# david-jk/BigGAN-Tensorflow

Measured on AMD Instinct MI355X. Metric: BigGAN-128 train-step images/sec, higher is better.
Workload: dtype bf16; 1 GPU; BigGAN-128 ch=96 bf16 (BASELINE config 3: global batch 256, 32/GPU over 8 GPUs); img_size=128, ch=96, per_gpu_batch=256, global_batch=256, da_policy=full, g_regularization=ortho_cosine, n_labels=0, gan_type=hinge, hip_graph=False, precision=bf16, parallelism=dp1

## Files before the change

### biggan-tensorflow_amd/csrc/igemm16.hip

```cpp
#include <stdlib.h>

#include "common.h"
#include "igemm.h"
#include "igemm16.h"
#include <type_traits>
#include "igemm_dev.h"

namespace bg {

typedef float f32x4_t __attribute__((ext_vector_type(4)));
typedef float f32x16_t __attribute__((ext_vector_type(16)));
typedef __bf16 bf16x8_t __attribute__((ext_vector_type(8)));
typedef short s16x4v __attribute__((ext_vector_type(4)));
typedef short s16x8v __attribute__((ext_vector_type(8)));
typedef __attribute__((address_space(3))) void lds_void_t;
typedef __attribute__((address_space(1))) const void gbl_void_t;
typedef __attribute__((address_space(3))) s16x4v lds_s16x4v;

__device__ uint4 g_zero_page[1024];

__device__ __forceinline__ void glds16(const void* src, unsigned char* lds_wave_base) {
    __builtin_amdgcn_global_load_lds((gbl_void_t*)src, (lds_void_t*)lds_wave_base, 16, 0, 0);
}

__device__ __forceinline__ void glds16_asm(const void* src, uint32_t lds_byte_addr) {
    unsigned keep;
    const uint32_t dst = __builtin_amdgcn_readfirstlane(lds_byte_addr);
    asm volatile("s_mov_b32 %0, m0\n\ts_mov_b32 m0, %2\n\ts_nop 0\n\tglobal_load_lds_dwordx4 %1, off\n\ts_mov_b32 m0, %0"
                 : "=&s"(keep)
                 : "v"(src), "s"(dst)
                 : "memory");
}

__device__ __forceinline__ uint32_t pack_bf16x2(float a, float b) {
    typedef __bf16 bf16x2_t __attribute__((ext_vector_type(2)));
    bf16x2_t v;
    v[0] = (__bf16)a;
    v[1] = (__bf16)b;
    return __builtin_bit_cast(uint32_t, v);
}
__device__ __forceinline__ float bf16_lo(uint32_t u) { return __builtin_bit_cast(float, u << 16); }
__device__ __forceinline__ float bf16_hi(uint32_t u) { return __builtin_bit_cast(float, u & 0xffff0000u); }

constexpr int NN16_BM = 128;
constexpr int NN16_TAPS = 4;
constexpr int NN16_RING_TAPS = 8;
constexpr int nn16_lds_bytes(int TN, int TAPS = NN16_TAPS) {
    const int stage = (NN16_BM + 32 * TN) * 128;
    const int epi = NN16_BM * (32 * TN + 4) * 4;
    const int tab = 2 * TAPS * NN16_BM * 4;
    return (2 * stage + tab > epi ? 2 * stage + tab : epi) + NN16_BM * 4 + 16;
}
constexpr int nn16_pipe_lds_bytes(int TN, int WM, int TAPS = NN16_TAPS) {
    const int bm = 64 * WM;
    return 3 * (bm + 32 * TN) * 64 + TAPS * bm * (4 + 2) + bm * 4 + 16;
}
constexpr int NN16_NOSRC = -(1 << 30);

template <int MODE>
__device__ __forceinline__ int64_t nn16_src_off(const Gather& g, const RowPos& r, int kh, int kw) {
    int h, w;
    if (MODE == GATHER_CONV) {
        h = conv_src(r.ho, kh, g.stride, g.pad, g.reflect, g.Hs);
        w = conv_src(r.wo, kw, g.stride, g.pad, g.reflect, g.Ws);
    } else {
        h = tconv_src_from_num(r.ho + g.pad - kh, g.stride, g.Hs);
        w = tconv_src_from_num(r.wo + g.pad - kw, g.stride, g.Ws);
    }
    const bool ok = r.valid && h >= 0 && w >= 0;
    const int pix = (r.b * g.Hs + h) * g.Ws + w;
    return ok ? (int64_t)pix * g.ld : (int64_t)-1;
}

constexpr int NN16_NOMIRROR = -(1 << 20);
__device__ __forceinline__ int nn16_mirror_pos(int o, int n, bool hi) {
    return o == 1 ? -1 : ((hi && o == n - 2) ? n : NN16_NOMIRROR);
}

template <int MODE, bool PM, bool RING = false>
__device__ __forceinline__ RowPos nn16_row(const NN16Params& p, int m, int ph, int pw) {
    RowPos r;
    if (PM) {
        r.valid = m < p.M;
        const int pos = m / p.g.Nb;
        r.b = m - pos * p.g.Nb;
        if (RING) {
            const int L = p.ring_lines, first = L * p.g.Wo;
            if (pos < first) {
                const int line = pos / p.g.Wo;
                r.ho = line == 0 ? 1 : p.g.Ho - 2;
                r.wo = pos - line * p.g.Wo;
            } else {
                const int per = p.g.Ho - L, q = pos - first;
                const int line = q / per, idx = q - line * per;
                r.wo = line == 0 ? 1 : p.g.Wo - 2;
                r.ho = idx == 0 ? 0 : ((L == 2 && idx > p.g.Ho - 4) ? p.g.Ho - 1 : idx + 1);
            }
            return r;
        }
        const int hq = pos / p.g.Wq;
        r.ho = hq * p.g.pstep + ph;
        r.wo = (pos - hq * p.g.Wq) * p.g.pstep + pw;
        return r;
    }
    if (MODE == GATHER_PLAIN || !p.pow2) return decompose_row<MODE>(p.g, m, p.M, ph, pw);
    r.valid = m < p.M;
    const int wq = m & (p.g.Wq - 1);
    const int t = m >> p.wq_shift;
    const int hq = t & (p.g.Hq - 1);
    r.b = t >> p.hq_shift;
    r.ho = hq * p.g.pstep + ph;
    r.wo = wq * p.g.pstep + pw;
    return r;
}

template <int TN, int MODE, bool PM, bool RING = false, int SLOTS = 2, int WM = 2>
__global__ __launch_bounds__(128 * WM, SLOTS == 2 ? 2 : (WM == 4 ? 4 : 3)) void nn16_kernel(const NN16Params p) {
    static_assert(!RING || (PM && MODE == GATHER_TCONV), "ring launches are position-major transposed gathers");
    static_assert((SLOTS == 2 && WM == 2) || (SLOTS == 3 && (WM == 2 || WM == 4)), "two stages, or a 3-slot ring on 4 / 8 waves");
    constexpr bool PIPE = SLOTS == 3;
    constexpr int TAPS = RING ? NN16_RING_TAPS : NN16_TAPS;
    constexpr int LDS_BYTES = PIPE ? nn16_pipe_lds_bytes(TN, WM, TAPS) : nn16_lds_bytes(TN, TAPS);
    typedef typename std::conditional<RING, uint64_t, unsigned>::type mask_t;
    typedef typename std::conditional<PIPE, int16_t, int>::type tabw_t;
    constexpr int BM = 64 * WM, BN = 32 * TN, NTHR = 128 * WM, NWV = 2 * WM;
    constexpr int CPS = PIPE ? 4 : 8;
    constexpr int ROWB = 16 * CPS;
    constexpr int RSTR = PIPE ? 16 * NWV : 32;
    constexpr int JA = BM / RSTR, JB = PIPE ? (BN / 16 + NWV - 1) / NWV : BN / 32;
    constexpr int A_BYTES = BM * ROWB, STAGE = (BM + BN) * ROWB;
    static_assert(BM == NN16_BM || PIPE, "the two-stage form has 128-row tiles");
    static_assert(A_BYTES % 1024 == 0 && STAGE % 1024 == 0 && (RSTR * ROWB) % 1024 == 0,
                  "every LDS-DMA destination is 1 KB aligned");
    static_assert(!PIPE || 64 * (BN + 4) * 4 <= SLOTS * STAGE, "a 64-row part of the epilogue fits in front of the tables");
    static_assert(!PIPE || RING || LDS_BYTES * (WM == 4 ? 2 : 3) <= 160 * 1024, "ring forms: 3 (8 waves: 2) blocks per CU");
    static_assert(!PIPE || LDS_BYTES * 2 <= 160 * 1024, "mirrored-tap ring launches: 2 blocks per CU");
    extern __shared__ __attribute__((aligned(16))) unsigned char smem[];

    const int t = threadIdx.x;
    const int lane = t & 63, w = PIPE ? __builtin_amdgcn_readfirstlane(t >> 6) : t >> 6;
    const int wm = w >> 1, wn = w & 1;
    const Gather& g = p.g;

    int tile_m, tile_n, bz = blockIdx.z;
    if (p.zfold > 0) {
        const int lin = xcd_remap(blockIdx.x, p.tiles_m * p.tiles_n * p.zfold);
        if (p.mfast) {
            tile_m = lin % p.tiles_m;
            const int r_ = lin / p.tiles_m;
            bz = r_ % p.zfold;
            tile_n = r_ / p.zfold;
        } else {
            bz = lin % p.zfold;
            const int tile = lin / p.zfold;
            tile_n = tile % p.tiles_n;
            tile_m = tile / p.tiles_n;
        }
    } else {
        const int tile = xcd_remap(blockIdx.x, p.tiles_m * p.tiles_n);
        if (p.mfast) {
            tile_m = tile % p.tiles_m;
            tile_n = tile / p.tiles_m;
        } else {
            tile_n = tile % p.tiles_n;
            tile_m = tile / p.tiles_n;
        }
    }
    const int m0 = tile_m * BM, n0 = tile_n * BN;
    const int zs = bz % p.splitk, zo = bz / p.splitk;

    int ph = 0, pw = 0;
    if (MODE == GATHER_TCONV) {
        ph = g.pstep - 1 - zo / g.pstep;
        pw = g.pstep - 1 - zo % g.pstep;
    }
    int kh0 = 0, kw0 = 0, kstep = 1, nkh = g.k, nkw = g.k;
    if (MODE == GATHER_TCONV && g.pstep > 1) {
        kstep = g.stride;
        kh0 = (ph + g.pad) % g.stride;
        kw0 = (pw + g.pad) % g.stride;
        nkh = (g.k - kh0 + g.stride - 1) / g.stride;
        nkw = (g.k - kw0 + g.stride - 1) / g.stride;
    }
    int nrh = 0, nrw = 0;
    if (RING) {
        nrh = nrw = g.k;
        nkh = nkw = 2 * g.k;
    }
    const int C8 = p.C >> 3;
    const int ntap = nkh * nkw;

    unsigned& s_any = *reinterpret_cast<unsigned*>(smem + LDS_BYTES - 16);
    if (PM) {
        if (t == 0) s_any = 0;
        __syncthreads();
    }
    unsigned any_local = 0;
    int* tabh = reinterpret_cast<int*>(smem + SLOTS * STAGE);
    tabw_t* tabw = reinterpret_cast<tabw_t*>(tabh + TAPS * BM);
    for (int e = t; e < 2 * TAPS * BM; e += NTHR) {
        const int axis = e / (TAPS * BM), i = (e / BM) % TAPS, row = e % BM;
        const RowPos r = nn16_row<MODE, PM, RING>(p, m0 + row, ph, pw);
        int v = NN16_NOSRC;
        if (r.valid && i < (axis ? nkw : nkh)) {
            int kk = (axis ? kw0 : kh0) + i * kstep;
            int o = axis ? r.wo : r.ho;
            const int n = axis ? g.Ws : g.Hs;
            if (RING) {
                const int nr = axis ? nrw : nrh;
                if (i >= nr) {
                    kk = i - nr;
                    o = nn16_mirror_pos(o, axis ? g.Wo : g.Ho, p.ring_lines == 2);
                }
            }
            const int src = MODE == GATHER_CONV ? conv_src(o, kk, g.stride, g.pad, g.reflect, n)
                                                : (o == NN16_NOMIRROR ? -1 : tconv_src_from_num(o + g.pad - kk, g.stride, n));
            if (src >= 0) {
                v = axis ? src : (r.b * g.Hs + src) * g.Ws;
                any_local |= 1u << (axis * TAPS + i);
            }
        }
        if (PIPE && axis) tabw[e - TAPS * BM] = (tabw_t)(v < 0 ? -1 : v);
        else tabh[e] = v;
    }
    if (PM && any_local) atomicOr(&s_any, any_local);
    unsigned* tabo = reinterpret_cast<unsigned*>(smem + LDS_BYTES - 16 - BM * 4);
    constexpr bool use_tabo = MODE == GATHER_TCONV || PM;
    if (use_tabo && t < BM) {
        const RowPos r = nn16_row<MODE, PM, RING>(p, m0 + t, ph, pw);
        tabo[t] = (r.valid && r.ho < g.Ho && r.wo < g.Wo) ? (unsigned)((r.b * g.Ho + r.ho) * g.Wo + r.wo) : 0xffffffffu;
    }

    const int cch = PIPE ? (lane & 3) ^ ((lane >> 3) & 2) : (lane & 7) ^ ((((w & 1) << 2) | (lane >> 4)) & 7);
    const int rsub = PIPE ? 16 * w + (lane >> 2) : 8 * w + (lane >> 3);
    constexpr int NB_HI = JB, NB_LO = (BN / 16) / NWV;
    const int nbw = (PIPE && NB_HI != NB_LO) ? (BN / 16 - w + NWV - 1) / NWV : JB;
    const unsigned char* abase = reinterpret_cast<const unsigned char*>(p.A);
    const unsigned char* bbase = reinterpret_cast<const unsigned char*>(p.B);
    const unsigned char* zero = reinterpret_cast<const unsigned char*>(g_zero_page);
    const unsigned ald2 = 2u * (unsigned)g.ld;
    const uint32_t lds0 = static_cast<uint32_t>(
        reinterpret_cast<uintptr_t>((__attribute__((address_space(3))) unsigned char*)smem));

    __syncthreads();
    mask_t tapmask = 0;
    if (PM) {
        const unsigned any = __builtin_amdgcn_readfirstlane(s_any);
        for (int i = 0; i < nkh; ++i)
            for (int j = 0; j < nkw; ++j)
                if (((any >> i) & (any >> (TAPS + j)) & 1u) != 0 && !(RING && i < nrh && j < nrw))
                    tapmask |= (mask_t)1 << (i * TAPS + j);
    }
    const int nsteps_all = ((PM ? __builtin_popcountll((uint64_t)tapmask) : ntap) * C8 + 7) >> 3;
    const int sps = (nsteps_all + p.splitk - 1) / p.splitk;
    const int it0 = zs * sps;
    const int nsteps = max(0, min(nsteps_all, it0 + sps) - it0);

    mask_t rem = tapmask;
    int tidx = 0, c8, ih = 0, iw = 0;
    {
        const int kk = it0 * 8 + cch;
        tidx = kk / C8;
        c8 = kk - tidx * C8;
        if (PM) {
            for (int i = 0; i < tidx && rem; ++i) rem &= rem - 1;
        } else {
            ih = tidx / nkw;
            iw = tidx - ih * nkw;
        }
    }
    const unsigned char* asrc[JA];
    const unsigned char* wsrc[JB];
    auto set_tap = [&]() {
        bool kvalid;
        if (PM) {
            kvalid = rem != 0;
            const int bit = kvalid ? __builtin_ctzll((uint64_t)rem) : 0;
            ih = bit / TAPS;
            iw = bit % TAPS;
        } else {
            kvalid = tidx < ntap;
        }
        const int* th = tabh + (ih & (TAPS - 1)) * BM + rsub;
        const tabw_t* tw = tabw + (iw & (TAPS - 1)) * BM + rsub;
#pragma unroll
        for (int j = 0; j < JA; ++j) {
            int col = tw[RSTR * j];
            if (PIPE) col = col < 0 ? NN16_NOSRC : col;
            const int pix = th[RSTR * j] + col;
            asrc[j] = (kvalid & (pix >= 0)) ? abase + (uint64_t)(unsigned)pix * ald2 : zero;
        }
        const int kh = RING ? (ih >= nrh ? ih - nrh : ih) : kh0 + ih * kstep;
        const int kw = RING ? (iw >= nrw ? iw - nrw : iw) : kw0 + iw * kstep;
        const unsigned char* wt = bbase + 2 * (int64_t)(kh * g.k + kw) * p.tap_stride;
#pragma unroll
        for (int j = 0; j < JB; ++j) {
            const int n = n0 + RSTR * j + rsub;
            wsrc[j] = (kvalid & (n < p.N)) ? wt + 2 * (uint64_t)((unsigned)n * (unsigned)p.C) : zero;
        }
    };
    set_tap();
    auto advance = [&]() {
        c8 += CPS;
        if (c8 >= C8) {
            do {
                c8 -= C8;
                if (PM) {
                    rem &= rem - 1;
                } else {
                    ++tidx;
                    if (++iw == nkw) {
                        iw = 0;
                        ++ih;
                    }
                }
            } while (c8 >= C8);
            set_tap();
        }
    };

    auto stage = [&](int buf) {
        const uint32_t sa = lds0 + buf * STAGE + w * 1024;
        const uint32_t sb = sa + A_BYTES;
        const unsigned cbyte = 16u * (unsigned)c8;
#pragma unroll
        for (int j = 0; j < JA; ++j) glds16_asm(asrc[j] + cbyte, sa + j * RSTR * ROWB);
#pragma unroll
        for (int j = 0; j < JB; ++j)
            if (!PIPE || j < nbw) glds16_asm(wsrc[j] + cbyte, sb + j * RSTR * ROWB);
        advance();
    };

    f32x4_t acc[4][TN];
#pragma unroll
    for (int i = 0; i < 4; ++i)
#pragma unroll
        for (int j = 0; j < TN; ++j)
#pragma unroll
            for (int r = 0; r < 4; ++r) acc[i][j][r] = 0.f;

    if constexpr (PIPE) {
        const int frag = (lane & 15) * ROWB + 16 * ((lane >> 4) ^ (((lane & 15) >> 1) & 2));
        const unsigned char* a_ad = smem + wm * 64 * ROWB + frag;
        const unsigned char* b_ad = smem + A_BYTES + wn * 16 * TN * ROWB + frag;
        const int nst = 2 * nsteps;
        if (nst > 0) stage(0);
        if (nst > 1) stage(1);
        auto kstep = [&](int it, auto slot_c) {
            constexpr int SLOT = decltype(slot_c)::value;
            if (it + 1 < nst) {
                if (NB_HI == NB_LO || nbw == NB_HI) asm volatile("s_waitcnt vmcnt(%0) lgkmcnt(0)" ::"n"(JA + NB_HI) : "memory");
                else asm volatile("s_waitcnt vmcnt(%0) lgkmcnt(0)" ::"n"(JA + NB_LO) : "memory");
            } else
                asm volatile("s_waitcnt vmcnt(0) lgkmcnt(0)" ::: "memory");
            __builtin_amdgcn_s_barrier();
            if (it + 2 < nst) stage((SLOT + 2) % 3);
            bf16x8_t a[4], b[TN];
#pragma unroll
            for (int i = 0; i < 4; ++i) a[i] = *reinterpret_cast<const bf16x8_t*>(a_ad + SLOT * STAGE + i * 16 * ROWB);
#pragma unroll
            for (int j = 0; j < TN; ++j) b[j] = *reinterpret_cast<const bf16x8_t*>(b_ad + SLOT * STAGE + j * 16 * ROWB);
#pragma unroll
            for (int i = 0; i < 4; ++i)
#pragma unroll
                for (int j = 0; j < TN; ++j)
                    acc[i][j] = __builtin_amdgcn_mfma_f32_16x16x32_bf16(b[j], a[i], acc[i][j], 0, 0, 0);
        };
        for (int it = 0; it < nst; it += 3) {
            kstep(it, std::integral_constant<int, 0>());
            if (it + 1 < nst) kstep(it + 1, std::integral_constant<int, 1>());
            if (it + 2 < nst) kstep(it + 2, std::integral_constant<int, 2>());
        }
        __syncthreads();
    } else {
    const int fsw = (lane & 15) >> 1;
    const int a_row = (wm * 64 + (lane & 15)) * 128;
    const int b_row = A_BYTES + (wn * 16 * TN + (lane & 15)) * 128;
    int koff[2];
#pragma unroll
    for (int s2 = 0; s2 < 2; ++s2) koff[s2] = 16 * ((4 * s2 + (lane >> 4)) ^ fsw);

    if (nsteps > 0) stage(0);
    asm volatile("s_waitcnt vmcnt(0) lgkmcnt(0)" ::: "memory");
    __builtin_amdgcn_s_barrier();

    for (int it = 0; it < nsteps; ++it) {
        const int cur = it & 1;
        if (it + 1 < nsteps) stage(cur ^ 1);
        const unsigned char* sbuf = smem + cur * STAGE;
        bf16x8_t a[2][4], b[2][TN];
#pragma unroll
        for (int s2 = 0; s2 < 2; ++s2) {
#pragma unroll
            for (int i = 0; i < 4; ++i)
                a[s2][i] = *reinterpret_cast<const bf16x8_t*>(sbuf + a_row + i * 16 * 128 + koff[s2]);
#pragma unroll
            for (int j = 0; j < TN; ++j)
                b[s2][j] = *reinterpret_cast<const bf16x8_t*>(sbuf + b_row + j * 16 * 128 + koff[s2]);
        }
#pragma unroll
        for (int s2 = 0; s2 < 2; ++s2)
#pragma unroll
            for (int i = 0; i < 4; ++i)
#pragma unroll
                for (int j = 0; j < TN; ++j)
                    acc[i][j] = __builtin_amdgcn_mfma_f32_16x16x32_bf16(b[s2][j], a[s2][i], acc[i][j], 0, 0, 0);
        asm volatile("s_waitcnt vmcnt(0) lgkmcnt(0)" ::: "memory");
        __builtin_amdgcn_s_barrier();
    }
    }

    constexpr int PARTS = PIPE ? WM : 1, PR = BM / PARTS;
    constexpr int ELD = BN + 4;
    float* est = reinterpret_cast<float*>(smem);
    const bool partial = p.splitk > 1;
    const float alpha = (!partial && p.alpha) ? *p.alpha : 1.0f;
    constexpr int CPR = BN / 8;
    float* slab = partial ? p.slabs + (int64_t)zs * p.slab_stride : nullptr;
#pragma unroll
    for (int part = 0; part < PARTS; ++part) {
    if (part > 0) __syncthreads();
    if (!PIPE || wm == part) {
#pragma unroll
        for (int i = 0; i < 4; ++i)
#pragma unroll
            for (int j = 0; j < TN; ++j) {
                const int row = (PIPE ? 0 : wm * 64) + 16 * i + (lane & 15);
                const int col = wn * 16 * TN + 16 * j + 4 * (lane >> 4);
                f32x4_t v = acc[i][j];
                v[0] *= alpha; v[1] *= alpha; v[2] *= alpha; v[3] *= alpha;
                *reinterpret_cast<f32x4_t*>(est + row * ELD + col) = v;
            }
    }
    __syncthreads();
#pragma unroll
    for (int q = 0; q < (PR * CPR + NTHR - 1) / NTHR; ++q) {
        const int idx = t + NTHR * q;
        if ((PR * CPR) % NTHR != 0 && idx >= PR * CPR) continue;
        const int erow = idx / CPR, cc = idx - erow * CPR;
        const int row = part * PR + erow;
        const int m = m0 + row, col = n0 + cc * 8;
        if (m >= p.M || col >= p.N) continue;
        int64_t ooff;
        if (use_tabo) {
            const unsigned op = tabo[row];
            if (op == 0xffffffffu) continue;
            ooff = (int64_t)op * p.out_ld + col;
        } else if (p.d2s_c) {
            int b, ho, wo;
            if (p.pow2) {
                wo = m & (g.Wo - 1);
                const int t2 = m >> p.wq_shift;
                ho = t2 & (g.Ho - 1);
                b = t2 >> p.hq_shift;
            } else {
                const int t2 = m / g.Wo;
                wo = m - t2 * g.Wo;
                b = t2 / g.Ho;
                ho = t2 - b * g.Ho;
            }
            const int sub = col / p.d2s_c, c = col - sub * p.d2s_c;
            ooff = (((int64_t)b * (2 * g.Ho) + 2 * ho + (sub >> 1)) * (2 * g.Wo) + 2 * wo + (sub & 1)) * p.d2s_c + c;
        } else {
            ooff = (int64_t)m * p.out_ld + col;
        }
        f32x4_t v0 = *reinterpret_cast<const f32x4_t*>(est + erow * ELD + cc * 8);
        f32x4_t v1 = *reinterpret_cast<const f32x4_t*>(est + erow * ELD + cc * 8 + 4);
        if (partial) {
            *reinterpret_cast<f32x4_t*>(slab + ooff) = v0;
            *reinterpret_cast<f32x4_t*>(slab + ooff + 4) = v1;
            continue;
        }
        if (p.bias) {
            const f32x4_t b0 = *reinterpret_cast<const f32x4_t*>(p.bias + col);
            const f32x4_t b1 = *reinterpret_cast<const f32x4_t*>(p.bias + col + 4);
            v0 += b0;
            v1 += b1;
        }
        if (p.out_f32) {
            float* o = reinterpret_cast<float*>(p.out) + ooff;
            if (p.accumulate) {
                v0 += *reinterpret_cast<const f32x4_t*>(o);
                v1 += *reinterpret_cast<const f32x4_t*>(o + 4);
            }
            *reinterpret_cast<f32x4_t*>(o) = v0;
            *reinterpret_cast<f32x4_t*>(o + 4) = v1;
        } else {
            __bf16* o = reinterpret_cast<__bf16*>(p.out) + ooff;
            if (p.accumulate) {
                const uint4 r = *reinterpret_cast<const uint4*>(o);
                v0[0] += bf16_lo(r.x); v0[1] += bf16_hi(r.x); v0[2] += bf16_lo(r.y); v0[3] += bf16_hi(r.y);
                v1[0] += bf16_lo(r.z); v1[1] += bf16_hi(r.z); v1[2] += bf16_lo(r.w); v1[3] += bf16_hi(r.w);
            }
            uint4 r;
            r.x = pack_bf16x2(v0[0], v0[1]);
            r.y = pack_bf16x2(v0[2], v0[3]);
            r.z = pack_bf16x2(v1[0], v1[1]);
            r.w = pack_bf16x2(v1[2], v1[3]);
            *reinterpret_cast<uint4*>(o) = r;
        }
    }
    }
}

__global__ __launch_bounds__(256) void nn16_slab_reduce_kernel(const float* __restrict__ slabs, void* __restrict__ out,
// ... 840 lines not shown
}

struct NN16Plan {
    int tn, splitk;
};

static int nn16_steps_min(const NN16Params& p, int mode) {
    int per_axis = p.g.k;
    if (mode == GATHER_TCONV && p.g.pstep > 1) per_axis = max(1, p.g.k / p.g.stride);
    return (per_axis * per_axis * (p.C >> 3) + 7) >> 3;
}

static double nn16_axis_fraction(const Gather& g, int mode, int nq, int n_src) {
    int64_t valid = 0, slots = 0;
    for (int ph = 0; ph < (mode == GATHER_TCONV ? g.pstep : 1); ++ph) {
        int k0 = 0, kstep = 1, nk = g.k;
        if (mode == GATHER_TCONV && g.pstep > 1) {
            kstep = g.stride;
            k0 = (ph + g.pad) % g.stride;
            nk = (g.k - k0 + g.stride - 1) / g.stride;
        }
        for (int q = 0; q < nq; ++q) {
            const int o = q * g.pstep + ph;
            for (int i = 0; i < nk; ++i) {
                const int kk = k0 + i * kstep;
                bool ok;
                if (mode == GATHER_CONV) {
                    const int src = o * g.stride + kk - g.pad;
                    ok = g.reflect || (src >= 0 && src < n_src);
                } else {
                    const int hn = o + g.pad - kk;
                    ok = hn >= 0 && hn % g.stride == 0 && hn / g.stride < n_src;
                }
                valid += ok;
            }
            slots += nk;
        }
    }
    return slots ? (double)valid / (double)slots : 1.0;
}

static double nn16_posmajor_fraction(const NN16Params& p, int mode) {
    const char* e = getenv("BG_NN16_POSMAJOR");
    if (e && atoi(e) == 0) return 1.0;
    const Gather& g = p.g;
    if (g.k <= 1 || g.Nb < 16 || g.Hq <= 0 || g.Wq <= 0 || (int64_t)g.Hq * g.Wq > 40 * 40) return 1.0;
    const double f = nn16_axis_fraction(g, mode, g.Hq, g.Hs) * nn16_axis_fraction(g, mode, g.Wq, g.Ws);
    return f < 0.9 ? f : 1.0;
}

static NN16Plan plan_nn16(const NN16Params& p, int mode, int zdim, bool allow_split) {
    static const int slots = getenv("BG_NN16_SLOTS") ? atoi(getenv("BG_NN16_SLOTS")) : 512;
    const int64_t tm = (p.M + NN16_BM - 1) / NN16_BM;
    int steps = nn16_steps_min(p, mode);
    const double pm = nn16_posmajor_fraction(p, mode);
    if (pm < 1.0) steps = max(1, (int)(steps * pm + 0.5));
    NN16Plan best{4, 1};
    double best_cost = 1e30;
    for (int tn = 4; tn >= 1; --tn) {
        const int bn = 32 * tn;
        const int64_t tiles = tm * ((p.N + bn - 1) / bn) * zdim;
        const double unit = 1.5 + tn;
        const int max_sk = allow_split ? (steps / 4 < 16 ? (steps / 4 < 1 ? 1 : steps / 4) : 16) : 1;
        for (int sk = 1; sk <= max_sk; ++sk) {
            const int64_t rounds = (tiles * sk + slots - 1) / slots;
            double cost = (double)rounds * ((steps + sk - 1) / sk + 2.0) * unit;
            if (sk > 1) cost += 6.0 * unit + 0.02 * sk * (double)tiles / slots * bn;
            if (cost < best_cost - 1e-9) {
                best_cost = cost;
                best = NN16Plan{tn, sk};
            }
        }
    }
    return best;
}

size_t nn16_workspace_bytes(const NN16Params& p, int mode, int zdim, int64_t out_elems) {
    const NN16Plan pl = plan_nn16(p, mode, zdim, true);
    return pl.splitk > 1 ? (size_t)pl.splitk * out_elems * sizeof(float) : 0;
}

static int nn16_mfast(const NN16Params& p, int tiles_m, int tiles_n);

enum { NN16_FORM_TWO = 0, NN16_FORM_RING = 1, NN16_FORM_WIDE = 2 };
static int nn16_form(const NN16Params& p, int tn, int64_t wide_blocks, bool mirrored) {
    if (p.g.Ws >= (1 << 15)) return NN16_FORM_TWO;
    const bool wide_ok = !mirrored && !p.posmajor;
    if (const char* e = getenv("BG_NN16_PIPE")) {
        const int v = atoi(e);
        if (v == 2) return wide_ok ? NN16_FORM_WIDE : NN16_FORM_TWO;
        return v == 1 ? NN16_FORM_RING : NN16_FORM_TWO;
    }
    return (wide_ok && p.C <= 192 && tn >= 2 && wide_blocks >= 512) ? NN16_FORM_WIDE : NN16_FORM_TWO;
}

template <int TN, int SLOTS = 2>
static int launch_nn16_ring_inst(const NN16Params& p, dim3 grid, hipStream_t s) {
    constexpr int lds = SLOTS == 3 ? nn16_pipe_lds_bytes(TN, 2, NN16_RING_TAPS) : nn16_lds_bytes(TN, NN16_RING_TAPS);
    if (!lds_opt_in(reinterpret_cast<const void*>(&nn16_kernel<TN, GATHER_TCONV, true, true, SLOTS>), lds)) return BG_ERR_LAUNCH;
    hipLaunchKernelGGL((nn16_kernel<TN, GATHER_TCONV, true, true, SLOTS>), grid, dim3(256), lds, s, p);
    return BG_OK;
}
template <int TN>
static int launch_nn16_ring_tn(const NN16Params& p, int form, dim3 grid, hipStream_t s) {
    return form == NN16_FORM_RING ? launch_nn16_ring_inst<TN, 3>(p, grid, s) : launch_nn16_ring_inst<TN>(p, grid, s);
}

int launch_nn16_ring(NN16Params& p, hipStream_t s) {
    BG_REQUIRE(p.ring == 1 && (p.ring_lines == 1 || p.ring_lines == 2), "nn16 ring launch: ring = 1, ring_lines 1 or 2");
    BG_REQUIRE(p.g.k >= 1 && p.g.k <= NN16_RING_TAPS / 2 && p.g.Ho >= 4 && p.g.Wo >= 4 && p.accumulate == 1,
               "nn16 ring launch: kernel size %d / map %d x %d not supported", p.g.k, p.g.Ho, p.g.Wo);
    BG_REQUIRE(p.C % 8 == 0 && p.N % 8 == 0 && p.g.ld % 8 == 0 && p.out_ld % 8 == 0, "nn16 ring launch: channels %% 8");
    const int npos = p.ring_lines * p.g.Wo + p.ring_lines * (p.g.Ho - p.ring_lines);
    p.g.pstep = 1;
    p.g.Hq = 1;
    p.g.Wq = npos;
    p.M = p.g.Nb * npos;
    p.posmajor = 1;
    p.splitk = 1;
    p.slabs = nullptr;
    p.zfold = 0;
    p.pow2 = 0;
    int tn = 4, best = 1 << 30;
    for (int c = 4; c >= 1; --c) {
        const int padded = (p.N + 32 * c - 1) / (32 * c) * (32 * c);
        if (padded < best) { best = padded; tn = c; }
    }
    p.tiles_m = (p.M + NN16_BM - 1) / NN16_BM;
    p.tiles_n = (p.N + 32 * tn - 1) / (32 * tn);
    p.mfast = nn16_mfast(p, p.tiles_m, p.tiles_n);
    dim3 grid(p.tiles_m * p.tiles_n, 1, 1);
    const int form = nn16_form(p, tn, 0, true);
    int rc;
    switch (tn) {
        case 1: rc = launch_nn16_ring_tn<1>(p, form, grid, s); break;
        case 2: rc = launch_nn16_ring_tn<2>(p, form, grid, s); break;
        case 3: rc = launch_nn16_ring_tn<3>(p, form, grid, s); break;
        default: rc = launch_nn16_ring_tn<4>(p, form, grid, s); break;
    }
    if (rc) return rc;
    BG_LAUNCH_CHECK();
    return BG_OK;
}

template <int TN, int MODE, bool PM, int SLOTS = 2, int WM = 2>
static int launch_nn16_inst(const NN16Params& p, dim3 grid, hipStream_t s) {
    constexpr int lds = SLOTS == 3 ? nn16_pipe_lds_bytes(TN, WM) : nn16_lds_bytes(TN);
    if (!lds_opt_in(reinterpret_cast<const void*>(&nn16_kernel<TN, MODE, PM, false, SLOTS, WM>), lds)) return BG_ERR_LAUNCH;
    if (SLOTS == 2) prof_kernel("nn16_kernel<%d, %d, %s>", TN, MODE, PM ? "true" : "false");
    else prof_kernel("nn16_kernel<%d, %d, %s, false, %d, %d>", TN, MODE, PM ? "true" : "false", SLOTS, WM);
    hipLaunchKernelGGL((nn16_kernel<TN, MODE, PM, false, SLOTS, WM>), grid, dim3(128 * WM), lds, s, p);
    return BG_OK;
}

template <int TN, int MODE, bool PM>
static int launch_nn16_tn(const NN16Params& p, int form, dim3 grid, hipStream_t s) {
    if (form == NN16_FORM_RING) return launch_nn16_inst<TN, MODE, PM, 3, 2>(p, grid, s);
    if constexpr (!PM)
        if (form == NN16_FORM_WIDE) return launch_nn16_inst<TN, MODE, PM, 3, 4>(p, grid, s);
    return launch_nn16_inst<TN, MODE, PM>(p, grid, s);
}

template <int MODE, bool PM>
static int launch_nn16_pm(const NN16Params& p, int tn, int form, dim3 grid, hipStream_t s) {
    switch (tn) {
        case 1: return launch_nn16_tn<1, MODE, PM>(p, form, grid, s);
        case 2: return launch_nn16_tn<2, MODE, PM>(p, form, grid, s);
        case 3: return launch_nn16_tn<3, MODE, PM>(p, form, grid, s);
        default: return launch_nn16_tn<4, MODE, PM>(p, form, grid, s);
    }
}

template <int MODE>
static int launch_nn16_mode(const NN16Params& p, int tn, int form, dim3 grid, hipStream_t s) {
    return p.posmajor ? launch_nn16_pm<MODE, true>(p, tn, form, grid, s) : launch_nn16_pm<MODE, false>(p, tn, form, grid, s);
}

static int nn16h_taps(const NN16Params& p, int mode, int zdim) {
    const char* e = getenv("BG_NN16_HALO");
    const int use = e ? atoi(e) : 1;
    static const int cmax = getenv("BG_NN16_HALO_CMAX") ? atoi(getenv("BG_NN16_HALO_CMAX")) : 4096;
    const Gather& g = p.g;
    if (!use || p.C > cmax || p.C % 32 || p.N % 8 || g.Hq < NH_T || g.Wq < NH_T || g.Hq % NH_T || g.Wq % NH_T) return 0;
    if (mode == GATHER_CONV) return (g.stride == 1 && g.k == 3 && g.pstep == 1 && zdim == 1) ? 3 : 0;
    if (g.reflect) return 0;
    if (g.stride == 1 && g.k == 3 && g.pstep == 1 && zdim == 1) return 3;
    if (g.stride == 2 && g.k == 4 && g.pstep == 2 && zdim == 4) return 2;
    if (g.stride == 2 && g.k == 3 && g.pad == 1 && g.pstep == 2 && zdim == 4) {
        const char* e3 = getenv("BG_NN16_HALO_K3S2");
        return (e3 && atoi(e3) == 1) ? 2 : 0;
    }
    return 0;
}

template <int NT, int NF, int MODE, int THIN = 0>
static int launch_nn16h_inst(const NN16Params& p, int blocks, hipStream_t s) {
    constexpr int lds = nn16h_lds_bytes<NT, NF>();
    if (!lds_opt_in(reinterpret_cast<const void*>(&nn16h_kernel<NT, NF, MODE, THIN>), lds)) return BG_ERR_LAUNCH;
    if (THIN) prof_kernel("nn16h_kernel<%d, %d, %d, d2s>", NT, NF, MODE);
    else prof_kernel("nn16h_kernel<%d, %d, %d>", NT, NF, MODE);
    hipLaunchKernelGGL((nn16h_kernel<NT, NF, MODE, THIN>), dim3(blocks), dim3(512), lds, s, p);
    return BG_OK;
}

template <int NT, int MODE>
static int launch_nn16h_nf(const NN16Params& p, int nf, int blocks, hipStream_t s) {
    switch (nf) {
        case 1: return launch_nn16h_inst<NT, 1, MODE>(p, blocks, s);
        case 2: return launch_nn16h_inst<NT, 2, MODE>(p, blocks, s);
        case 3: return launch_nn16h_inst<NT, 3, MODE>(p, blocks, s);
        default: return launch_nn16h_inst<NT, 4, MODE>(p, blocks, s);
    }
}

bool nn16h_d2s_ok(const NN16Params& p) {
    const char* e = getenv("BG_THIN_D2S");
    const int use = e ? atoi(e) : 1;
    const Gather& g = p.g;
    return use && p.N == 8 && p.out_ld == 8 && g.k == 3 && g.stride == 2 && g.pad == 1 && !g.reflect && p.C % 32 == 0 &&
           g.Hs % NH_T == 0 && g.Ws % NH_T == 0 && g.Ho == 2 * g.Hs && g.Wo == 2 * g.Ws && !p.bias && !p.stats_part;
}
int launch_nn16h_d2s(const NN16Params& plain, hipStream_t s) {
    BG_REQUIRE(nn16h_d2s_ok(plain), "nn16h depth-to-space form: unsupported geometry");
    NN16Params p = plain;
    Gather& g = p.g;
    g.Hq = g.Hs; g.Wq = g.Ws; g.pstep = 1; g.pad = 0; g.stride = 1;
    p.N = 32;
    p.splitk = 1; p.mfast = 0; p.ring = 0;
    const int64_t blocks = (int64_t)g.Nb * (g.Hq / NH_T) * (g.Wq / NH_T);
    BG_REQUIRE(blocks > 0 && blocks < (int64_t(1) << 31), "nn16h: grid out of range");
    if (const int rc = launch_nn16h_inst<2, 1, GATHER_CONV, 1>(p, (int)blocks, s)) return rc;
    BG_LAUNCH_CHECK();
    return BG_OK;
}

static int nn16_mfast(const NN16Params& p, int tiles_m, int tiles_n) {
    const char* e = getenv("BG_NN16_MFAST");
    if (!e) return 0;
    if (strcmp(e, "auto") != 0) return atoi(e) != 0;
    const double l2 = 3.0e6;
    const double a_bytes = 2.0 * p.g.Nb * (double)p.g.Hs * p.g.Ws * p.g.ld;
    const double w_bytes = 2.0 * p.g.k * p.g.k * (double)p.N * p.C;
    const double nfast = a_bytes + (w_bytes > l2 ? w_bytes * tiles_m : w_bytes);
    const double mfast = w_bytes + (a_bytes > l2 ? a_bytes * tiles_n : a_bytes);
    return mfast < nfast;
}

static int launch_nn16h(NN16Params& p, int mode, int ntaps, hipStream_t s) {
    int nf = 4, best = 1 << 30;
    for (int c = 4; c >= 1; --c) {
        const int padded = (p.N + 32 * c - 1) / (32 * c) * (32 * c);
        if (padded < best) { best = padded; nf = c; }
    }
    const Gather& g = p.g;
    const int64_t blocks = (int64_t)g.Nb * (g.Hq / NH_T) * (g.Wq / NH_T) * ((p.N + 32 * nf - 1) / (32 * nf)) *
                           (g.pstep * g.pstep);
    BG_REQUIRE(blocks > 0 && blocks < (int64_t(1) << 31), "nn16h: grid out of range");
    p.splitk = 1;
    p.mfast = nn16_mfast(p, g.Nb * (g.Hq / NH_T) * (g.Wq / NH_T), (p.N + 32 * nf - 1) / (32 * nf));
    int rc;
    if (mode == GATHER_CONV) rc = launch_nn16h_nf<3, GATHER_CONV>(p, nf, (int)blocks, s);
    else if (ntaps == 3) rc = launch_nn16h_nf<3, GATHER_TCONV>(p, nf, (int)blocks, s);
    else rc = launch_nn16h_nf<2, GATHER_TCONV>(p, nf, (int)blocks, s);
    if (rc) return rc;
    BG_LAUNCH_CHECK();
    return BG_OK;
}

bool nn16_d2s_ok(const NN16Params& p, int mode, int zdim) {
    const Gather& g = p.g;
    if (p.d2s_c <= 0 || p.d2s_c % 8 || p.N != 4 * p.d2s_c || p.C % 8 || mode != GATHER_CONV || zdim != 1 || g.stride != 1 ||
        g.pstep != 1 || g.Hq != g.Ho || g.Wq != g.Wo || p.stats_part || p.ring)
        return false;
    if ((int64_t)g.Nb * g.Ho * g.Wo * 4 >= (int64_t(1) << 31)) return false;
    if (nn16h_taps(p, mode, zdim)) return true;
    if (nn16_posmajor_fraction(p, mode) < 1.0) return false;
    return plan_nn16(p, mode, zdim, true).splitk == 1;
}

int64_t nn16_stats_rows(const NN16Params& p, int mode, int zdim) {
    if (p.C % 8 || p.N % 8 || !nn16h_taps(p, mode, zdim)) return 0;
    return 2 * (int64_t)p.g.Nb * (p.g.Hq / NH_T) * (p.g.Wq / NH_T) * (p.g.pstep * p.g.pstep);
}

int launch_nn16(NN16Params& p, int mode, int zdim, int64_t out_elems, void* ws, size_t ws_bytes, hipStream_t s) {
    BG_REQUIRE(p.C % 8 == 0 && p.N % 8 == 0 && p.g.ld % 8 == 0 && p.out_ld % 8 == 0,
               "bf16-resident conv: channel counts must be multiples of 8 (C=%d N=%d)", p.C, p.N);
    BG_REQUIRE((reinterpret_cast<uintptr_t>(p.A) & 15) == 0 && (reinterpret_cast<uintptr_t>(p.B) & 15) == 0 &&
                   (reinterpret_cast<uintptr_t>(p.out) & 15) == 0,
               "bf16-resident conv: tensors must be 16-byte aligned");
    BG_REQUIRE(p.g.k >= 1 && p.g.k <= NN16_TAPS && p.C <= 8192 && p.g.stride >= 1 && p.g.stride <= 2,
               "bf16-resident conv: kernel size %d / stride %d / %d channels not supported", p.g.k, p.g.stride, p.C);
    BG_REQUIRE((int64_t)p.g.Nb * p.g.Hs * p.g.Ws < (int64_t(1) << 30) && (int64_t)p.g.Nb * p.g.Ho * p.g.Wo < (int64_t(1) << 31),
               "bf16-resident conv: more than 2^30 source / 2^31 output pixels");
    BG_REQUIRE(p.d2s_c == 0 || (nn16_d2s_ok(p, mode, zdim) && ws == nullptr),
               "bf16-resident conv: this launch has no depth-to-space store (bg_conv2d_fwd_d2s_supported)");
    if (const int ntaps = nn16h_taps(p, mode, zdim)) return launch_nn16h(p, mode, ntaps, s);
    BG_REQUIRE(p.stats_part == nullptr, "bf16-resident conv: fused statistics need the halo-tile form (nn16_stats_rows)");
    NN16Plan pl = plan_nn16(p, mode, zdim, ws != nullptr);
    if (pl.splitk > 1 && ws_bytes < (size_t)pl.splitk * out_elems * sizeof(float)) pl.splitk = 1;
    p.splitk = pl.splitk;
    p.slabs = reinterpret_cast<float*>(ws);
    p.slab_stride = out_elems;
    const int bn = 32 * pl.tn;
    p.tiles_n = (p.N + bn - 1) / bn;
    p.posmajor = nn16_posmajor_fraction(p, mode) < 1.0;
    const int form = nn16_form(p, pl.tn, (int64_t)((p.M + 255) / 256) * p.tiles_n * zdim * pl.splitk, false);
    const int bm = form == NN16_FORM_WIDE ? 256 : NN16_BM;
    p.tiles_m = (p.M + bm - 1) / bm;
    p.pow2 = 0;
    if (p.g.Wq > 0 && p.g.Hq > 0 && (p.g.Wq & (p.g.Wq - 1)) == 0 && (p.g.Hq & (p.g.Hq - 1)) == 0) {
        p.pow2 = 1;
        p.wq_shift = __builtin_ctz(p.g.Wq);
        p.hq_shift = __builtin_ctz(p.g.Hq);
    }
    p.mfast = nn16_mfast(p, p.tiles_m, p.tiles_n);
    dim3 grid(p.tiles_m * p.tiles_n, 1, zdim * p.splitk);
    p.zfold = 0;
    if (mode == GATHER_TCONV && zdim > 1 && p.splitk == 1 && p.g.k % p.g.stride == 0) {
        p.zfold = zdim;
        grid = dim3(p.tiles_m * p.tiles_n * zdim, 1, 1);
    }
    int rc;
    if (mode == GATHER_CONV)
        rc = launch_nn16_mode<GATHER_CONV>(p, pl.tn, form, grid, s);
    else
        rc = launch_nn16_mode<GATHER_TCONV>(p, pl.tn, form, grid, s);
    if (rc) return rc;
    BG_LAUNCH_CHECK();
    if (pl.splitk > 1) {
        const int64_t n8 = out_elems / 8;
        int blocks = (int)((n8 + 255) / 256);
        if (blocks > 2048) blocks = 2048;
        hipLaunchKernelGGL(nn16_slab_reduce_kernel, dim3(blocks), dim3(256), 0, s, p.slabs, p.out, p.bias, p.alpha, n8,
                           p.N, pl.splitk, out_elems, p.accumulate, p.out_f32);
        BG_LAUNCH_CHECK();
    }
    return BG_OK;
}

static void plan_tn16(TN16Params& p) {
    const int64_t tiles = (int64_t)((p.Mf + 127) / 128) * ((p.Cb + 127) / 128);
    static const int want = getenv("BG_TN16_WANT") ? atoi(getenv("BG_TN16_WANT")) : 1024;
    int sk = (int)(want / tiles);
    const int max_sk = (p.M + 4 * TN16_BK - 1) / (4 * TN16_BK);
    if (sk > max_sk) sk = max_sk;
    if (sk < 1) sk = 1;
    if (sk > 512) sk = 512;
    int rps = (p.M + sk - 1) / sk;
    rps = (rps + TN16_BK - 1) / TN16_BK * TN16_BK;
    p.splitk = (p.M + rps - 1) / rps;
    p.rows_per_split = rps;
}

static int tn16x_nbi(const TN16Params& p) {
    const char* e = getenv("BG_TN16X_NBI");
    if (!e || atoi(e) != 2) return 1;
    return (p.Cb >= 512 && p.Cb % 256 == 0 && p.Mf >= 256) ? 2 : 1;
}

static bool plan_tn16x(const TN16Params& p, int* sk_out, int* rps_out) {
    static const int use_wide = getenv("BG_TN16_WIDE") ? atoi(getenv("BG_TN16_WIDE")) : 1;
    if (!use_wide || p.Mf <= 128 || p.M < 8 * TN16_BK) return false;
    if (p.g.k > 0 && (p.g.Wq <= 0 || p.g.Hq <= 0 || (p.g.Wq & (p.g.Wq - 1)) || (p.g.Hq & (p.g.Hq - 1)))) return false;
    const int nbi = tn16x_nbi(p);
    const int tm = (p.Mf + 255) / 256, tn = (p.Cb + 128 * nbi - 1) / (128 * nbi);
    static const int wantx0 = getenv("BG_TN16X_WANT") ? atoi(getenv("BG_TN16X_WANT")) : 512;
    const int wantx = nbi == 2 ? wantx0 / 2 : wantx0;
    int sk = wantx / (tm * tn);
    const int max_sk = (p.M + 4 * TN16_BK - 1) / (4 * TN16_BK);
    if (sk > max_sk) sk = max_sk;
    if (sk < 1) sk = 1;
    if (sk > 512) sk = 512;
    int rps = (p.M + sk - 1) / sk;
    rps = (rps + TN16_BK - 1) / TN16_BK * TN16_BK;
    *sk_out = (p.M + rps - 1) / rps;
    *rps_out = rps;
    return true;
}

size_t tn16_workspace_bytes(const TN16Params& p0) {
    TN16Params p = p0;
    plan_tn16(p);
    int sk = p.splitk, skx = 1, rps = 0;
    if (plan_tn16x(p0, &skx, &rps) && skx > sk) sk = skx;
    return sk > 1 ? (size_t)sk * p.Mf * p.Cb * sizeof(float) : 0;
}

int launch_tn16(TN16Params& p, int mode, float* final_out, void* ws, size_t ws_bytes, hipStream_t s) {
    BG_REQUIRE(p.Ca % 8 == 0 && p.Cb % 8 == 0 && p.g.ld % 8 == 0 && p.b_ld % 8 == 0,
               "bf16-resident wgrad: channel counts must be multiples of 8 (Ca=%d Cb=%d)", p.Ca, p.Cb);
    BG_REQUIRE((reinterpret_cast<uintptr_t>(p.A) & 15) == 0 && (reinterpret_cast<uintptr_t>(p.Bv) & 15) == 0,
               "bf16-resident wgrad: tensors must be 16-byte aligned");
    plan_tn16(p);
    const int64_t total = (int64_t)p.Mf * p.Cb;
    if (p.splitk > 1 && (ws == nullptr || ws_bytes < (size_t)p.splitk * total * sizeof(float) || p.out_ld != p.Cb)) {
        p.splitk = 1;
        p.rows_per_split = (p.M + TN16_BK - 1) / TN16_BK * TN16_BK;
    }
    if (p.splitk > 1) {
        p.out = reinterpret_cast<float*>(ws);
        p.slab_stride = total;
    } else {
        p.out = final_out;
        p.slab_stride = 0;
    }
    p.tiles_m = (p.Mf + 127) / 128;
    p.tiles_n = (p.Cb + 127) / 128;
    p.pow2 = 0;
    if (mode != GATHER_PLAIN && (p.g.Wq & (p.g.Wq - 1)) == 0 && (p.g.Hq & (p.g.Hq - 1)) == 0) {
// ... 77 lines not shown
```

Before: 2682 images/sec.

## Add phased 256-row, 8-wave conv GEMM form with quadrant-interleaved loads

Adds a new 'phased' variant of the bf16 implicit-GEMM conv kernel. It uses 256-row tiles with 128, 192 or 256 columns on 8 waves and one block per CU. Each K-step is split into four MFMA quadrants, and the LDS-DMA loads for the next stage are interleaved between them. Barriers and s_setprio keep the loads and MFMAs overlapped. A heuristic in nn16_form selects this form when channel counts are large and the block count divides evenly across 256 CUs. The aim is better MFMA utilisation and data reuse on large convs, at the cost of lower occupancy and more complex, fragile wait-count logic.

New measurement: 2744 images/sec, median of 6. 1.02x the previous value.

```diff
diff --git a/biggan-tensorflow_amd/csrc/igemm16.hip b/biggan-tensorflow_amd/csrc/igemm16.hip
--- a/biggan-tensorflow_amd/csrc/igemm16.hip
+++ b/biggan-tensorflow_amd/csrc/igemm16.hip
@@ -54,6 +54,9 @@
 constexpr int nn16_pipe_lds_bytes(int TN, int WM, int TAPS = NN16_TAPS) {
     const int bm = 64 * WM;
     return 3 * (bm + 32 * TN) * 64 + TAPS * bm * (4 + 2) + bm * 4 + 16;
+}
+constexpr int nn16x_lds_bytes(int TN) {
+    return 2 * (256 + 32 * TN) * 128 + 2 * NN16_TAPS * 256 * 4 + 256 * 4 + 16;
 }
 constexpr int NN16_NOSRC = -(1 << 30);
 
@@ -117,19 +120,25 @@
 template <int TN, int MODE, bool PM, bool RING = false, int SLOTS = 2, int WM = 2>
 __global__ __launch_bounds__(128 * WM, SLOTS == 2 ? 2 : (WM == 4 ? 4 : 3)) void nn16_kernel(const NN16Params p) {
     static_assert(!RING || (PM && MODE == GATHER_TCONV), "ring launches are position-major transposed gathers");
-    static_assert((SLOTS == 2 && WM == 2) || (SLOTS == 3 && (WM == 2 || WM == 4)), "two stages, or a 3-slot ring on 4 / 8 waves");
+    static_assert((SLOTS == 2 && (WM == 2 || WM == 4)) || (SLOTS == 3 && (WM == 2 || WM == 4)),
+                  "two stages (WM = 4: the phased form), or a 3-slot ring on 4 / 8 waves");
     constexpr bool PIPE = SLOTS == 3;
+    constexpr bool PHASED = SLOTS == 2 && WM == 4;
+    static_assert(!PHASED || (!RING && (TN == 4 || TN == 6 || TN == 8)), "phased form: 128, 192 or 256 columns, no mirrored taps");
+    static_assert(PHASED || TN <= 4, "tiles of at most 128 columns");
     constexpr int TAPS = RING ? NN16_RING_TAPS : NN16_TAPS;
-    constexpr int LDS_BYTES = PIPE ? nn16_pipe_lds_bytes(TN, WM, TAPS) : nn16_lds_bytes(TN, TAPS);
+    constexpr int LDS_BYTES = PIPE ? nn16_pipe_lds_bytes(TN, WM, TAPS) : (PHASED ? nn16x_lds_bytes(TN) : nn16_lds_bytes(TN, TAPS));
     typedef typename std::conditional<RING, uint64_t, unsigned>::type mask_t;
     typedef typename std::conditional<PIPE, int16_t, int>::type tabw_t;
     constexpr int BM = 64 * WM, BN = 32 * TN, NTHR = 128 * WM, NWV = 2 * WM;
     constexpr int CPS = PIPE ? 4 : 8;
     constexpr int ROWB = 16 * CPS;
-    constexpr int RSTR = PIPE ? 16 * NWV : 32;
-    constexpr int JA = BM / RSTR, JB = PIPE ? (BN / 16 + NWV - 1) / NWV : BN / 32;
+    constexpr int RSTR = PIPE ? 16 * NWV : 8 * NWV;
+    constexpr int JA = BM / RSTR, JB = PIPE ? (BN / 16 + NWV - 1) / NWV : (PHASED ? 2 * ((BN / 2 + 63) / 64) : BN / RSTR);
     constexpr int A_BYTES = BM * ROWB, STAGE = (BM + BN) * ROWB;
-    static_assert(BM == NN16_BM || PIPE, "the two-stage form has 128-row tiles");
+    static_assert(BM == NN16_BM || PIPE || PHASED, "the two-stage form has 128-row tiles");
+    static_assert(!PHASED || (LDS_BYTES <= 160 * 1024 && 128 * (BN + 4) * 4 <= LDS_BYTES - 16 - BM * 4),
+                  "phased form: one block per CU; a 128-row part of the epilogue ends in front of tabo");
     static_assert(A_BYTES % 1024 == 0 && STAGE % 1024 == 0 && (RSTR * ROWB) % 1024 == 0,
                   "every LDS-DMA destination is 1 KB aligned");
     static_assert(!PIPE || 64 * (BN + 4) * 4 <= SLOTS * STAGE, "a 64-row part of the epilogue fits in front of the tables");
@@ -138,7 +147,7 @@
     extern __shared__ __attribute__((aligned(16))) unsigned char smem[];
 
     const int t = threadIdx.x;
-    const int lane = t & 63, w = PIPE ? __builtin_amdgcn_readfirstlane(t >> 6) : t >> 6;
+    const int lane = t & 63, w = (PIPE || PHASED) ? __builtin_amdgcn_readfirstlane(t >> 6) : t >> 6;
     const int wm = w >> 1, wn = w & 1;
     const Gather& g = p.g;
 
@@ -295,8 +304,10 @@
         const unsigned char* wt = bbase + 2 * (int64_t)(kh * g.k + kw) * p.tap_stride;
 #pragma unroll
         for (int j = 0; j < JB; ++j) {
-            const int n = n0 + RSTR * j + rsub;
-            wsrc[j] = (kvalid & (n < p.N)) ? wt + 2 * (uint64_t)((unsigned)n * (unsigned)p.C) : zero;
+            const int brow = PHASED ? (BN / 2) * (j / (JB / 2)) + 64 * (j % (JB / 2)) + rsub : RSTR * j + rsub;
+            const bool inside = !PHASED || 64 * (j % (JB / 2)) + rsub < BN / 2;
+            const int n = n0 + brow;
+            wsrc[j] = (kvalid & inside & (n < p.N)) ? wt + 2 * (uint64_t)((unsigned)n * (unsigned)p.C) : zero;
         }
     };
     set_tap();
@@ -331,13 +342,27 @@
         advance();
     };
 
-    f32x4_t acc[4][TN];
-#pragma unroll
-    for (int i = 0; i < 4; ++i)
-#pragma unroll
-        for (int j = 0; j < TN; ++j)
-#pragma unroll
-            for (int r = 0; r < 4; ++r) acc[i][j][r] = 0.f;
+    constexpr int XMI = PHASED ? (TN == 8 ? 4 : 2) : 1, XNJ = PHASED ? (TN == 6 ? 3 : 2) : 1;
+    typedef f32x4_t acc_plain_t[4][TN];
+    typedef f32x4_t acc_quad_t[2][XMI][2][XNJ];
+    typename std::conditional<PHASED, acc_quad_t, acc_plain_t>::type accv;
+    auto& acc = accv;
+    auto& accx = accv;
+    if constexpr (PHASED) {
+#pragma unroll
+        for (int i = 0; i < 2 * XMI; ++i)
+#pragma unroll
+            for (int j = 0; j < 2 * XNJ; ++j)
+#pragma unroll
+                for (int r = 0; r < 4; ++r) accx[i / XMI][i % XMI][j / XNJ][j % XNJ][r] = 0.f;
+    } else {
+#pragma unroll
+        for (int i = 0; i < 4; ++i)
+#pragma unroll
+            for (int j = 0; j < TN; ++j)
+#pragma unroll
+                for (int r = 0; r < 4; ++r) acc[i][j][r] = 0.f;
+    }
 
     if constexpr (PIPE) {
         const int frag = (lane & 15) * ROWB + 16 * ((lane >> 4) ^ (((lane & 15) >> 1) & 2));
@@ -372,6 +397,136 @@
             if (it + 2 < nst) kstep(it + 2, std::integral_constant<int, 2>());
         }
         __syncthreads();
+    } else if constexpr (PHASED) {
+        constexpr int WNX = TN == 8 ? 4 : 2, JBH = JB / 2;
+        static_assert(JA == 4 && (8 / WNX) * XMI * 16 == 128 && WNX * XNJ * 16 == BN / 2, "halves of 128 rows / BN / 2 columns");
+        const int wmx = w / WNX, wnx = w % WNX;
+        const bool b_short = TN == 6 && w >= 4;
+        const int fsw = (lane & 15) >> 1;
+        const int a_row = (wmx * 16 * XMI + (lane & 15)) * 128;
+        const int b_row = A_BYTES + (wnx * 16 * XNJ + (lane & 15)) * 128;
+        int koff[2];
+#pragma unroll
+        for (int s2 = 0; s2 < 2; ++s2) koff[s2] = 16 * ((4 * s2 + (lane >> 4)) ^ fsw);
+        auto piece_a = [&](int buf, auto h_c) {
+            constexpr int H = decltype(h_c)::value;
+            const uint32_t sa = lds0 + buf * STAGE + w * 1024;
+            const unsigned cbyte = 16u * (unsigned)c8;
+#pragma unroll
+            for (int j = 2 * H; j < 2 * H + 2; ++j) glds16_asm(asrc[j] + cbyte, sa + j * RSTR * ROWB);
+        };
+        auto piece_b = [&](int buf, auto h_c) {
+            constexpr int H = decltype(h_c)::value;
+            const uint32_t sb = lds0 + buf * STAGE + w * 1024 + A_BYTES;
+            const unsigned cbyte = 16u * (unsigned)c8;
+#pragma unroll
+            for (int jj = 0; jj < JBH; ++jj)
+                if (jj == 0 || !b_short) glds16_asm(wsrc[JBH * H + jj] + cbyte, sb + ((BN / 2) * H + 64 * jj) * ROWB);
+        };
+        auto wait_fly = [&]() {
+            if (b_short) asm volatile("s_waitcnt vmcnt(%0)" ::"n"(2 * JBH) : "memory");
+            else asm volatile("s_waitcnt vmcnt(%0)" ::"n"(2 + 2 * JBH) : "memory");
+        };
+        const std::integral_constant<int, 0> c0;
+        const std::integral_constant<int, 1> c1;
+        auto read_a = [&](bf16x8_t (&a)[2][XMI], const unsigned char* sbuf, int h) {
+#pragma unroll
+            for (int s2 = 0; s2 < 2; ++s2)
+#pragma unroll
+                for (int i = 0; i < XMI; ++i)
+                    a[s2][i] = *reinterpret_cast<const bf16x8_t*>(sbuf + a_row + (128 * h + 16 * i) * 128 + koff[s2]);
+        };
+        auto read_b = [&](bf16x8_t (&b)[2][XNJ], const unsigned char* sbuf, int hn) {
+#pragma unroll
+            for (int s2 = 0; s2 < 2; ++s2)
+#pragma unroll
+                for (int j = 0; j < XNJ; ++j)
+                    b[s2][j] = *reinterpret_cast<const bf16x8_t*>(sbuf + b_row + ((BN / 2) * hn + 16 * j) * 128 + koff[s2]);
+        };
+        auto mid = [&]() {
+            __builtin_amdgcn_s_barrier();
+            asm volatile("s_waitcnt lgkmcnt(0)" ::: "memory");
+            __builtin_amdgcn_sched_barrier(0);
+            __builtin_amdgcn_s_setprio(1);
+        };
+        auto close = [&]() {
+            __builtin_amdgcn_s_setprio(0);
+            __builtin_amdgcn_sched_barrier(0);
+            __builtin_amdgcn_s_barrier();
+        };
+        auto quad = [&](auto h_c, auto hn_c, const bf16x8_t (&a)[2][XMI], const bf16x8_t (&b)[2][XNJ]) {
+            constexpr int H = decltype(h_c)::value, HN = decltype(hn_c)::value;
+#pragma unroll
+            for (int s2 = 0; s2 < 2; ++s2)
+#pragma unroll
+                for (int i = 0; i < XMI; ++i)
+#pragma unroll
+                    for (int j = 0; j < XNJ; ++j)
+                        accx[H][i][HN][j] = __builtin_amdgcn_mfma_f32_16x16x32_bf16(b[s2][j], a[s2][i], accx[H][i][HN][j], 0, 0, 0);
+        };
+        auto ktile = [&](int u, auto buf_c, auto tail_c) {
+            constexpr int BUF = decltype(buf_c)::value;
+            constexpr bool TAIL = decltype(tail_c)::value;
+            const unsigned char* sbuf = smem + BUF * STAGE;
+            const bool n1 = !TAIL || u + 1 < nsteps, n2 = !TAIL || u + 2 < nsteps;
+            bf16x8_t a[2][XMI], b0[2][XNJ], b1[2][XNJ];
+            read_b(b0, sbuf, 0);
+            __builtin_amdgcn_sched_barrier(0);
+            read_a(a, sbuf, 0);
+            if (n1) {
+                piece_a(BUF ^ 1, c1);
+                advance();
+            }
+            mid();
+            quad(c0, c0, a, b0);
+            close();
+            read_b(b1, sbuf, 1);
+            if (n2) piece_a(BUF, c0);
+            mid();
+            quad(c0, c1, a, b1);
+            close();
+            read_a(a, sbuf, 1);
+            if (n2) piece_b(BUF, c0);
+            mid();
+            quad(c1, c1, a, b1);
+            close();
+            if (n2) {
+                piece_b(BUF, c1);
+                wait_fly();
+            } else {
+                asm volatile("s_waitcnt vmcnt(0)" ::: "memory");
+            }
+            mid();
+            quad(c1, c0, a, b0);
+            close();
+        };
+        if (nsteps > 0) {
+            piece_a(0, c0);
+            piece_b(0, c0);
+            piece_b(0, c1);
+            piece_a(0, c1);
+            advance();
+        }
+        if (nsteps > 1) {
+            piece_a(1, c0);
+            piece_b(1, c0);
+            piece_b(1, c1);
+            wait_fly();
+            asm volatile("s_waitcnt lgkmcnt(0)" ::: "memory");
+        } else {
+            asm volatile("s_waitcnt vmcnt(0) lgkmcnt(0)" ::: "memory");
+        }
+        __builtin_amdgcn_s_barrier();
+        const std::integral_constant<bool, false> steady;
+        const std::integral_constant<bool, true> tail;
+        int u = 0;
+        for (; u + 4 <= nsteps; u += 2) {
+            ktile(u, c0, steady);
+            ktile(u + 1, c1, steady);
+        }
+        if (u < nsteps) ktile(u, c0, tail);
+        if (u + 1 < nsteps) ktile(u + 1, c1, tail);
+        if (u + 2 < nsteps) ktile(u + 2, c0, tail);
     } else {
     const int fsw = (lane & 15) >> 1;
     const int a_row = (wm * 64 + (lane & 15)) * 128;
@@ -410,7 +565,7 @@
     }
     }
 
-    constexpr int PARTS = PIPE ? WM : 1, PR = BM / PARTS;
+    constexpr int PARTS = PIPE ? WM : (PHASED ? 2 : 1), PR = BM / PARTS;
     constexpr int ELD = BN + 4;
     float* est = reinterpret_cast<float*>(smem);
     const bool partial = p.splitk > 1;
@@ -420,7 +575,20 @@
 #pragma unroll
     for (int part = 0; part < PARTS; ++part) {
     if (part > 0) __syncthreads();
-    if (!PIPE || wm == part) {
+    if constexpr (PHASED) {
+        constexpr int WNX = TN == 8 ? 4 : 2;
+        const int wmx = w / WNX, wnx = w % WNX;
+#pragma unroll
+        for (int i = 0; i < XMI; ++i)
+#pragma unroll
+            for (int hj = 0; hj < 2 * XNJ; ++hj) {
+                const int row = wmx * 16 * XMI + 16 * i + (lane & 15);
+                const int col = (BN / 2) * (hj / XNJ) + wnx * 16 * XNJ + 16 * (hj % XNJ) + 4 * (lane >> 4);
+                f32x4_t v = accx[part][i][hj / XNJ][hj % XNJ];
+                v[0] *= alpha; v[1] *= alpha; v[2] *= alpha; v[3] *= alpha;
+                *reinterpret_cast<f32x4_t*>(est + row * ELD + col) = v;
+            }
+    } else if (!PIPE || wm == part) {
 #pragma unroll
         for (int i = 0; i < 4; ++i)
 #pragma unroll
@@ -1427,15 +1595,34 @@
 
 static int nn16_mfast(const NN16Params& p, int tiles_m, int tiles_n);
 
-enum { NN16_FORM_TWO = 0, NN16_FORM_RING = 1, NN16_FORM_WIDE = 2 };
-static int nn16_form(const NN16Params& p, int tn, int64_t wide_blocks, bool mirrored) {
-    if (p.g.Ws >= (1 << 15)) return NN16_FORM_TWO;
-    const bool wide_ok = !mirrored && !p.posmajor;
+enum { NN16_FORM_TWO = 0, NN16_FORM_RING = 1, NN16_FORM_WIDE = 2, NN16_FORM_PHASED = 3 };
+constexpr int NN16X_CUS = 256;
+static int nn16_form(const NN16Params& p, int tn, int64_t row_blocks, bool even_phases, bool mirrored, int* xtn) {
+    const bool wide_ok = !mirrored && !p.posmajor && p.g.Ws < (1 << 15);
+    const bool phased_ok = !mirrored && (!p.posmajor || p.g.Nb % 256 == 0);
+    const int64_t wide_blocks = row_blocks * ((p.N + 32 * tn - 1) / (32 * tn));
+    const int64_t nb256 = row_blocks * ((p.N + 255) / 256), nb192 = row_blocks * ((p.N + 191) / 192);
+    const int64_t last192 = (nb192 + NN16X_CUS - 1) / NN16X_CUS * NN16X_CUS - nb192;
+    const int pad192 = (p.N + 191) / 192 * 192, pad_plan = (p.N + 32 * tn - 1) / (32 * tn) * (32 * tn);
+    int bn = 0;
+    if (phased_ok && p.C >= 384) {
+        if (p.N % 256 == 0 && nb256 % NN16X_CUS == 0 && even_phases) bn = 256;
+        else if (pad192 <= pad_plan && nb192 >= (even_phases ? 1 : 2) * NN16X_CUS && last192 * 16 <= NN16X_CUS) bn = 192;
+    }
+    const int rule_bn = bn;
+    if (bn == 0) bn = p.N <= 128 ? 128 : (p.N <= 192 ? 192 : 256);
+    if (const char* e = getenv("BG_NN16X_BN")) {
+        const int v = atoi(e);
+        if (v == 128 || v == 192 || v == 256) bn = v;
+    }
+    *xtn = bn / 32;
     if (const char* e = getenv("BG_NN16_PIPE")) {
         const int v = atoi(e);
+        if (v == 3) return phased_ok ? NN16_FORM_PHASED : NN16_FORM_TWO;
         if (v == 2) return wide_ok ? NN16_FORM_WIDE : NN16_FORM_TWO;
-        return v == 1 ? NN16_FORM_RING : NN16_FORM_TWO;
-    }
+        return (v == 1 && p.g.Ws < (1 << 15)) ? NN16_FORM_RING : NN16_FORM_TWO;
+    }
+    if (rule_bn) return NN16_FORM_PHASED;
     return (wide_ok && p.C <= 192 && tn >= 2 && wide_blocks >= 512) ? NN16_FORM_WIDE : NN16_FORM_TWO;
 }
 
@@ -1475,7 +1662,8 @@
     p.tiles_n = (p.N + 32 * tn - 1) / (32 * tn);
     p.mfast = nn16_mfast(p, p.tiles_m, p.tiles_n);
     dim3 grid(p.tiles_m * p.tiles_n, 1, 1);
-    const int form = nn16_form(p, tn, 0, true);
+    int xtn;
+    const int form = nn16_form(p, tn, 0, true, true, &xtn);
     int rc;
     switch (tn) {
         case 1: rc = launch_nn16_ring_tn<1>(p, form, grid, s); break;
@@ -1490,9 +1678,9 @@
 
 template <int TN, int MODE, bool PM, int SLOTS = 2, int WM = 2>
 static int launch_nn16_inst(const NN16Params& p, dim3 grid, hipStream_t s) {
-    constexpr int lds = SLOTS == 3 ? nn16_pipe_lds_bytes(TN, WM) : nn16_lds_bytes(TN);
+    constexpr int lds = SLOTS == 3 ? nn16_pipe_lds_bytes(TN, WM) : (WM == 4 ? nn16x_lds_bytes(TN) : nn16_lds_bytes(TN));
     if (!lds_opt_in(reinterpret_cast<const void*>(&nn16_kernel<TN, MODE, PM, false, SLOTS, WM>), lds)) return BG_ERR_LAUNCH;
-    if (SLOTS == 2) prof_kernel("nn16_kernel<%d, %d, %s>", TN, MODE, PM ? "true" : "false");
+    if (SLOTS == 2 && WM == 2) prof_kernel("nn16_kernel<%d, %d, %s>", TN, MODE, PM ? "true" : "false");
     else prof_kernel("nn16_kernel<%d, %d, %s, false, %d, %d>", TN, MODE, PM ? "true" : "false", SLOTS, WM);
     hipLaunchKernelGGL((nn16_kernel<TN, MODE, PM, false, SLOTS, WM>), grid, dim3(128 * WM), lds, s, p);
     return BG_OK;
@@ -1508,6 +1696,10 @@
 
 template <int MODE, bool PM>
 static int launch_nn16_pm(const NN16Params& p, int tn, int form, dim3 grid, hipStream_t s) {
+    if (form == NN16_FORM_PHASED)
+        return tn == 8   ? launch_nn16_inst<8, MODE, PM, 2, 4>(p, grid, s)
+               : tn == 6 ? launch_nn16_inst<6, MODE, PM, 2, 4>(p, grid, s)
+                         : launch_nn16_inst<4, MODE, PM, 2, 4>(p, grid, s);
     switch (tn) {
         case 1: return launch_nn16_tn<1, MODE, PM>(p, form, grid, s);
         case 2: return launch_nn16_tn<2, MODE, PM>(p, form, grid, s);
@@ -1647,11 +1839,14 @@
     p.splitk = pl.splitk;
     p.slabs = reinterpret_cast<float*>(ws);
     p.slab_stride = out_elems;
-    const int bn = 32 * pl.tn;
+    p.posmajor = nn16_posmajor_fraction(p, mode) < 1.0;
+    int xtn;
+    const int form = nn16_form(p, pl.tn, (int64_t)((p.M + 255) / 256) * zdim * pl.splitk,
+                               zdim == 1 || p.g.k % p.g.stride == 0, false, &xtn);
+    const int ltn = form == NN16_FORM_PHASED ? xtn : pl.tn;
+    const int bn = 32 * ltn;
     p.tiles_n = (p.N + bn - 1) / bn;
-    p.posmajor = nn16_posmajor_fraction(p, mode) < 1.0;
-    const int form = nn16_form(p, pl.tn, (int64_t)((p.M + 255) / 256) * p.tiles_n * zdim * pl.splitk, false);
-    const int bm = form == NN16_FORM_WIDE ? 256 : NN16_BM;
+    const int bm = (form == NN16_FORM_WIDE || form == NN16_FORM_PHASED) ? 256 : NN16_BM;
     p.tiles_m = (p.M + bm - 1) / bm;
     p.pow2 = 0;
     if (p.g.Wq > 0 && p.g.Hq > 0 && (p.g.Wq & (p.g.Wq - 1)) == 0 && (p.g.Hq & (p.g.Hq - 1)) == 0) {
@@ -1668,9 +1863,9 @@
     }
     int rc;
     if (mode == GATHER_CONV)
-        rc = launch_nn16_mode<GATHER_CONV>(p, pl.tn, form, grid, s);
+        rc = launch_nn16_mode<GATHER_CONV>(p, ltn, form, grid, s);
     else
-        rc = launch_nn16_mode<GATHER_TCONV>(p, pl.tn, form, grid, s);
+        rc = launch_nn16_mode<GATHER_TCONV>(p, ltn, form, grid, s);
     if (rc) return rc;
     BG_LAUNCH_CHECK();
     if (pl.splitk > 1) {
```
